# mulns/AccFlow

Measured on AMD Instinct MI355X. Metric: frame-pairs/s (estimator pair-evals/s), AccFlow(RAFT) 7-frame 480x1024 backward accumulation, higher is better.
Workload: dtype f32 (direct-kernel operands split into 2 fp16 terms - activations kept pre-split in HBM as fp16 hi+lo, 4 B per element; other kernels 3 bf16 terms; f32 accumulate)

## Files before the change

accflow_amd/_lib.py:

```python
import ctypes
import os
import threading

_HERE = os.path.dirname(os.path.abspath(__file__))
LIB_PATH = os.environ.get("ACCFLOW_HIP_LIB") or os.path.join(_HERE, "lib", "libaccflow_hip.so")

ABI_VERSION = 20
c_f = ctypes.c_void_p
c_ll = ctypes.c_longlong
c_i = ctypes.c_int


class ConvSrc(ctypes.Structure):
    _fields_ = [
        ("ptr", c_f), ("bs", c_ll),
        ("C", c_i), ("Hs", c_i), ("Ws", c_i),
        ("step", c_i), ("oy", c_i), ("ox", c_i),
        ("KH", c_i), ("KW", c_i), ("padH", c_i), ("padW", c_i),
        ("reserved", c_i),
    ]


MAX_SRC = 4

# ... 48 lines not shown
    "accflow_conv_pack_patch": [c_f, c_f, c_i, c_i, c_i, c_i, c_f, c_f],
    "accflow_conv_pack_patch16": [c_f, c_f, c_i, c_i, c_i, c_i, c_f, c_f, c_f],
    "accflow_conv_pack_split16": [c_f, c_f, c_i, c_i, c_i, c_i, c_f, c_f, c_f],
    "accflow_conv_multi_pack_elems": [c_i, c_i, ctypes.POINTER(c_i), ctypes.POINTER(c_i), ctypes.POINTER(c_i)],
    "accflow_conv_pack_multi16": [ctypes.POINTER(c_f), c_f, c_i, c_i, ctypes.POINTER(c_i), ctypes.POINTER(c_i), ctypes.POINTER(c_i),
                                  c_f, c_f, c_f],
    "accflow_conv2d_f32": [ctypes.POINTER(ConvDesc), c_f],
    "accflow_conv_stat_slots": [ctypes.POINTER(ConvDesc)],
    "accflow_conv_in_norm_supported": [ctypes.POINTER(ConvDesc)],
    "accflow_conv_plan_query": [ctypes.POINTER(ConvDesc), ctypes.POINTER(c_i), c_i],
    "accflow_conv_gru16_supported": [],
    "accflow_instance_stats_finalize_f32": [c_f, c_i, c_f, c_i, c_i, ctypes.c_float, c_f],
    "accflow_instance_norm_apply_f32": [c_f, c_f, c_i, c_f, c_f, c_f, c_i, c_i, c_i, ctypes.c_float, c_i, c_f],
    "accflow_instance_norm_apply_s16_f32": [c_f, c_f, c_i, c_f, c_f, c_f, c_f, c_ll, c_f, c_i, c_i, c_i, ctypes.c_float, c_i, c_f],
    "accflow_instance_norm_apply_s16res_f32": [c_f, c_f, c_i, c_f, c_f, c_ll, c_f, c_f, c_ll, c_f, c_i, c_i, c_i, ctypes.c_float, c_f],
    "accflow_instance_stats_finalize_sub_f32": [c_f, c_i, c_i, c_i, c_f, c_i, c_i, ctypes.c_float, c_f],
    "accflow_instance_norm_apply_s16proj_f32": [c_f, c_f, c_i, c_f, c_ll, c_f, c_i, c_i, c_i, c_f, c_f, c_ll, c_f, c_i, c_i, c_i,
                                                ctypes.c_float, c_f],
    "accflow_get_occ_s16": [c_f, c_ll, c_f, c_ll, c_f, c_ll, c_f, c_ll, c_f, c_i, c_i, c_i, c_i, c_i, c_f],
    "accflow_blend_s16": [c_f, c_f, c_f, c_f, c_ll, c_f, c_i, c_i, c_i, c_f],
    "accflow_deform_columns_s16": [c_f, c_ll, c_f, c_ll, c_f, c_ll, c_i, c_f, c_ll, c_f, c_i, c_i, c_i, c_i, c_i, c_i, c_i, c_i, c_f],
    "accflow_corr_volume_f32": [c_f, c_f, c_f, c_f, c_f, c_f, c_i, c_i, c_i, c_i, c_f],
    "accflow_corr_volume_ws_bytes": [c_i, c_i, c_i],
    "accflow_corr_volume_split_f32": [c_f, c_f, c_f, c_f, c_f, c_f, c_f, c_i, c_i, c_i, c_i, c_i, c_f],
    "accflow_corr_lookup_f32": [c_f, c_f, c_f, c_f, c_f, c_f, c_ll, c_i, c_i, c_i, c_f],
    "accflow_corr_disp_supported": [c_i, c_i],
    "accflow_corr_disp_level_elems": [c_i, c_i, c_i],
    "accflow_corr_volume_disp_f32": [c_f, c_f, c_f, c_f, c_f, c_f, c_f, c_i, c_f, c_i, c_i, c_i, c_i, c_f],
    "accflow_corr_pack_bytes": [c_i, c_i, c_i],
    "accflow_corr_pack_f32": [c_f, c_f, c_i, c_f, c_i, c_i, c_i, c_i, c_f],
    "accflow_corr_volume_disp_packed_f32": [c_f, c_i, ctypes.POINTER(c_i), ctypes.POINTER(c_i), c_f, c_f, c_f, c_f, c_i, c_f, c_i, c_i, c_i,
                                            c_i, c_f],
    "accflow_corr_disp_pool_f32": [c_f, c_f, c_f, c_f, c_i, c_i, c_i, c_f],
    "accflow_corr_lookup_disp_f32": [c_f, c_f, c_f, c_f, c_f, c_f, c_ll, c_i, c_i, c_i, c_f],
    "accflow_corr_lookup_disp_s16": [c_f, c_f, c_f, c_f, c_f, c_f, c_ll, c_f, c_i, c_i, c_i, c_f],
    "accflow_corr_alt_pyramid_elems": [c_i, c_i, c_i],
    "accflow_corr_alt_pyramid_f32": [c_f, c_f, c_i, c_i, c_i, c_i, c_f],
    "accflow_corr_lookup_alt_f32": [c_f, c_i, c_f, c_f, c_f, c_ll, c_i, c_i, c_i, c_i, c_f],
    "accflow_corr_lookup_alt_s16": [c_f, c_i, c_f, c_f, c_f, c_ll, c_f, c_i, c_i, c_i, c_i, c_f],
    "accflow_corr_lookup_convc1_kpad": [],
    "accflow_corr_lookup_convc1_s16": [c_f, c_f, c_f, c_f, c_f, c_f, c_f, c_f, c_f, c_ll, c_f, c_ll, c_i, c_f, c_i, c_i, c_i, c_i, c_f],
    "accflow_flow_from_coords_s16": [c_f, c_f, c_ll, c_f, c_ll, c_f, c_ll, c_f, c_ll, c_i, c_f, c_i, c_i, c_i, c_i, c_f],
    "accflow_convex_upsample_f32": [c_f, c_ll, c_f, c_ll, c_f, c_i, c_i, c_i, c_f],
    "accflow_backwarp_f32": [c_f, c_ll, c_f, c_ll, c_f, c_ll, c_i, c_i, c_i, c_i, c_f],
    "accflow_compose_flow_f32": [c_f, c_ll, c_f, c_ll, c_f, c_ll, c_i, c_i, c_i, c_f],
    "accflow_get_occ_f32": [c_f, c_ll, c_f, c_ll, c_f, c_ll, c_f, c_ll, c_i, c_i, c_i, c_i, c_i, c_f],
    "accflow_downflow8_f32": [c_f, c_f, c_i, c_i, c_i, c_i, c_f],
    "accflow_forward_interpolate_f32": [c_f, c_f, c_i, c_i, c_i, c_f],
    "accflow_instance_norm_f32": [c_f, c_f, c_f, c_i, c_i, c_i, ctypes.c_float, c_i, c_f],
    "accflow_split_tanh_relu_f32": [c_f, c_f, c_ll, c_f, c_ll, c_i, c_i, c_i, c_i, c_f],
    "accflow_split_tanh_relu_idx_f32": [c_f, c_i, ctypes.POINTER(c_i), c_f, c_ll, c_f, c_ll, c_i, c_i, c_i, c_i, c_f],
    "accflow_coords_grid_f32": [c_f, c_f, c_i, c_i, c_i, c_f],
    "accflow_flow_from_coords_f32": [c_f, c_f, c_ll, c_f, c_ll, c_f, c_i, c_i, c_i, c_i, c_f],
    "accflow_deform_columns_f32": [c_f, c_ll, c_f, c_ll, c_f, c_ll, c_f, c_i, c_i, c_i, c_i, c_i, c_i, c_i, c_i, c_f],
    "accflow_conv_pack_all_f32": [c_f, c_f, c_i, c_i, c_i, c_i, c_i, c_i, c_i, c_f, c_f, c_f, c_f, c_f, c_f, c_f, c_f],
    "accflow_tap_sum_f32": [c_f, c_f, c_f, c_ll, c_f, c_ll, c_i, c_i, c_i, c_i, c_i, c_i, c_i, c_i, c_i, c_i, c_f],
    "accflow_tap_sum_parts_f32": [c_f, c_i, c_ll, c_ll, c_f, c_f, c_ll, c_f, c_ll, c_i, c_i, c_i, c_i, c_i, c_i, c_i, c_i, c_i, c_i, c_f],
    "accflow_blend_f32": [c_f, c_f, c_f, c_f, c_i, c_i, c_i, c_f],
    "accflow_activation_f32": [c_f, c_ll, c_i, c_i, c_i, c_i, c_f],
    "accflow_copy_f32": [c_f, c_ll, c_f, c_ll, c_i, c_i, c_i, c_f],
    "accflow_gma_attention_f32": [c_f, c_f, c_i, c_i, c_i, ctypes.c_float, c_f],
    "accflow_gma_attention_ws_bytes": [c_i, c_i, c_i],
    "accflow_gma_attention_t_f32": [c_f, c_f, c_f, c_i, c_i, c_i, c_i, c_i, ctypes.c_float, c_f],
    "accflow_gma_aggregate_ws_bytes": [c_i, c_i, c_i],
    "accflow_gma_attention_s16_ws_bytes": [c_i, c_i, c_i],
    "accflow_gma_attention_s16": [c_f, c_f, c_f, c_f, c_i, c_i, c_i, c_i, ctypes.c_float, c_f],
# ... 59 lines not shown
```

accflow_amd/csrc/conv2d.hip:

```cpp
#include "conv_common.h"

namespace {

__global__ void conv_pack_patch_kernel(const float* __restrict__ w, const float* __restrict__ scale, int Cout, int Cin,
                                       int T, int CoutPad, unsigned short* __restrict__ wp, int f16,
                                       const float* __restrict__ wscale16, int octs = 2,
                                       const float* __restrict__ gptr = nullptr) {
  const int nstep = (Cin + 8 * octs - 1) / (8 * octs) * T;
  const long long per_term = (long long)nstep * octs * CoutPad * 8;
  const long long idx = (long long)blockIdx.x * blockDim.x + threadIdx.x;
  if (idx >= per_term) return;
  const int q = (int)(idx & 7);
  long long r = idx >> 3;
  const int ch = (int)(r % CoutPad); r /= CoutPad;
  const int o = (int)(r % octs); r /= octs;
  const int step = (int)r, cc = step / T, tap = step % T;
  const int c = cc * 8 * octs + o * 8 + q;
  float val = 0.0f;
  if (c < Cin && ch < Cout) {
    val = w[((long long)ch * Cin + c) * T + tap];
    if (scale) val *= scale[ch];
    if (gptr) val *= gptr[0];
  }
  float rr = val;
// ... 27 lines not shown
  const int k = (int)(idx / CoutPad), o = (int)(idx % CoutPad);
  const int T = KH * KW, K = Cin * T;
  float val = 0.0f;
  if (k < K && o < Cout) {
    const int c = k / T, t = k % T;
    val = kmajor ? w[(long long)k * Cout + o] : w[((long long)o * Cin + c) * T + t];
    if (scale) val *= scale[o];
    val *= cscale;
    if (gptr) val *= gptr[0];
  }
  const long long per_term = (long long)Kpad * CoutPad;
  const long long dst = ((long long)(k / 8) * CoutPad + o) * 8 + (k % 8);
  float r = val;
  if (wscale16) {
    r = val * (ldexpf(1.0f, -ACCFLOW_F16_ASHIFT) / wscale16[o]);
#pragma unroll
    for (int t = 0; t < 3; ++t) {
      const _Float16 hq = t < 2 ? (_Float16)r : (_Float16)0.0f;
      ws[t * per_term + dst] = __builtin_bit_cast(unsigned short, hq);
      r -= (float)hq;
    }
    return;
  }
#pragma unroll
  for (int t = 0; t < 3; ++t) {
    const __bf16 b = (__bf16)r;
    ws[t * per_term + dst] = __builtin_bit_cast(unsigned short, b);
    r -= (float)b;
  }
}

__global__ __launch_bounds__(256) void conv_pack_kmajor_kernel(const float* __restrict__ w, int Cout, int K, int Kpad,
                                                               int CoutPad, u32x4* __restrict__ ws, float cscale, int f16,
                                                               int* guard) {
  const long long idx = (long long)blockIdx.x * 256 + threadIdx.x;
  if (idx >= (long long)(Kpad / 8) * CoutPad) return;
  const int k8 = (int)(idx / CoutPad), o = (int)(idx % CoutPad);
  float x[8];
#pragma unroll
  for (int j = 0; j < 8; ++j) {
    const int k = k8 * 8 + j;
    x[j] = (k < K && o < Cout) ? w[(long long)k * Cout + o] * cscale : 0.0f;
  }
  const long long per_term = (long long)(Kpad / 8) * CoutPad;
  if (f16) {
    u32x4 t2[2];
    bool bad = false;
    split8_f16<0>(x, t2, bad, 1.0f);
    if (bad && guard) atomicOr(guard, 1);
    ws[idx] = t2[0];
    ws[per_term + idx] = t2[1];
  } else {
    u32x4 t3[3];
    split8_bf16<3, 0>(x, t3);
#pragma unroll
    for (int t = 0; t < 3; ++t) ws[t * per_term + idx] = t3[t];
  }
}

template <int CO>
__global__ __launch_bounds__(256) void conv2d_small_cout_kernel(const accflow_conv_desc d) {
  __shared__ float red[4][CO][64];
  const int tid = threadIdx.x, lane = tid & 63;
  const int q = __builtin_amdgcn_readfirstlane(tid >> 6);
  const int OHW = d.OH * d.OW;
  const int Ptot = d.B * OHW;
  const int p = blockIdx.x * 64 + lane;
  const bool pvalid = p < Ptot;
  const int pb = pvalid ? p / OHW : 0;
// ... 530 lines not shown
      d.in0 = reinterpret_cast<const float*>(bsplit);
      d.wpatch = wsplit;
      if (f16) { d.wpatch16 = wsplit; d.guard = guard; d.acc_scale = 1.0f / (fs * fs); }
      if (!lvl1) return 1;
      d.out2 = lvl1 + (long long)b * ((P + 127) / 128) * 128 * (H8 >> 1) * (W8 >> 1);
      const int rc = accflow_launch_corr_disp_direct(d, st);
      if (rc) return rc;
      if (lvl1_done) *lvl1_done = 1;
      continue;
    }
    if (disp) {
      const int rc = accflow_launch_corr_disp_bf16s(d, st);
      if (rc) return rc;
      continue;
    }
    const int rc = accflow_conv2d_f32(&d, st);
    if (rc) return rc;
  }
  return (int)hipGetLastError();
}

extern "C" long long accflow_corr_pack_bytes(int C, int H8, int W8) {
  return 3LL * accflow_conv_kpad(C, 1, 1) * accflow_conv_coutpad(H8 * W8) * 2;
}

extern "C" int accflow_corr_pack_f32(const float* fmaps, void* packs, int mode, int* guard, int F, int C, int H8, int W8,
                                     void* stream) {
  if (!fmaps || !packs || F <= 0 || C < 16 || (C % 16) || (W8 & 1) || !accflow_corr_disp_supported(H8, W8)) return 1;
  if (mode != ACCFLOW_CONV_BF16X3 && mode != ACCFLOW_CONV_BF16X6 && mode != ACCFLOW_CONV_F16X3) return 1;
  const int P = H8 * W8, Kpad = accflow_conv_kpad(C, 1, 1), CoutPad = accflow_conv_coutpad(P);
  const bool f16 = mode == ACCFLOW_CONV_F16X3;
  const float fs = f16 ? ldexpf(1.0f, ACCFLOW_F16_ASHIFT) : 1.0f;
  const long long n = (long long)Kpad * CoutPad, bytes = accflow_corr_pack_bytes(C, H8, W8);
  for (int f = 0; f < F; ++f)
    hipLaunchKernelGGL(conv_pack_kmajor_kernel, dim3(cdiv(n / 8, 256)), dim3(256), 0, as_stream(stream),
                       fmaps + (long long)f * C * P, P, C, Kpad, CoutPad,
                       reinterpret_cast<u32x4*>(reinterpret_cast<char*>(packs) + f * bytes), fs, f16 ? 1 : 0, guard);
  ACCFLOW_RETURN_LAUNCH_STATUS();
}

int accflow_corr_disp_pool_from(const float* lvl0, float* lvl1, float* lvl2, float* lvl3, int B, int H8, int W8, int first,
                                hipStream_t st);

extern "C" int accflow_corr_volume_disp_packed_f32(const void* packs, int F, const int* idx1, const int* idx2, float* lvl0,
                                                   float* lvl1, float* lvl2, float* lvl3, int mode, int* guard, int B,
                                                   int C, int H8, int W8, void* stream) {
  if (!packs || F <= 0 || !idx1 || !idx2 || !lvl0 || !lvl1 || !lvl2 || !lvl3 || B <= 0 || C < 16 || (C % 16) || (W8 & 1) ||
      !accflow_corr_disp_supported(H8, W8))
    return 1;
  for (int b = 0; b < B; ++b)
    if (idx1[b] < 0 || idx2[b] < 0 || idx1[b] >= F || idx2[b] >= F) return 1;
  if (mode != ACCFLOW_CONV_BF16X3 && mode != ACCFLOW_CONV_BF16X6 && mode != ACCFLOW_CONV_F16X3) return 1;
  hipStream_t st = as_stream(stream);
  const int P = H8 * W8, Kpad = accflow_conv_kpad(C, 1, 1), CoutPad = accflow_conv_coutpad(P);
  const bool f16 = mode == ACCFLOW_CONV_F16X3;
  const float fs = f16 ? ldexpf(1.0f, ACCFLOW_F16_ASHIFT) : 1.0f;
  const long long bytes = accflow_corr_pack_bytes(C, H8, W8);
  const long long pair0 = (long long)((P + 127) / 128) * 128 * P, pair1 = (long long)((P + 127) / 128) * 128 * (H8 >> 1) * (W8 >> 1);
  for (int b = 0; b < B; ++b) {
    const char* a = reinterpret_cast<const char*>(packs) + idx1[b] * bytes;
    const char* t = reinterpret_cast<const char*>(packs) + idx2[b] * bytes;
    accflow_conv_desc d = {};
    d.in0 = reinterpret_cast<const float*>(t);
    d.C0 = C; d.B = 1; d.H = H8; d.W = W8; d.OH = H8; d.OW = W8; d.KH = 1; d.KW = 1; d.stride = 1;
    d.Cout = P; d.Kpad = Kpad; d.CoutPad = CoutPad;
    d.out = lvl0 + b * pair0; d.out_bs = pair0; d.out2 = lvl1 + b * pair1;
    d.mode = mode; d.wpatch = a;
    if (f16) { d.wpatch16 = a; d.guard = guard; }
    d.acc_scale = (1.0f / sqrtf((float)C)) / (fs * fs);
    const int rc = accflow_launch_corr_disp_direct(d, st);
    if (rc) return rc;
  }
  return accflow_corr_disp_pool_from(lvl0, lvl1, lvl2, lvl3, B, H8, W8, 1, st);
}

int accflow_gma_aggregate_conv(const float* attnT, const float* v, const float* fmap, const float* gamma, float* out,
                               long long out_bs, void* ws, int mode, int* guard, int B, int D, int H, int W, hipStream_t st) {
  const int P = H * W;
  const int Kpad = accflow_conv_kpad(P, 1, 1), CoutPad = accflow_conv_coutpad(D);
  if (mode == ACCFLOW_CONV_F16X3 && B == 1 && P >= 16) {
    unsigned short* wpatch16 = reinterpret_cast<unsigned short*>(ws);
    float* wscale16 = reinterpret_cast<float*>(wpatch16 + accflow_conv_patch_elems(D, P, 1, 1));
    float* kws = wscale16 + CoutPad;
    const long long n = accflow_conv_patch_elems(D, P, 1, 1) / 3;
    hipLaunchKernelGGL(conv_row_scale16_kernel, dim3(CoutPad), dim3(256), 0, st, v, nullptr, D, P, wscale16, gamma);
    hipLaunchKernelGGL(conv_pack_patch_kernel, dim3(cdiv(n, 256)), dim3(256), 0, st, v, nullptr, D, P, 1, CoutPad, wpatch16, 1,
                       wscale16, 2, gamma);
    accflow_conv_desc d = {};
    d.in0 = attnT; d.in0_bs = (long long)P * P; d.C0 = P;
    d.B = 1; d.H = H; d.W = W; d.OH = H; d.OW = W; d.KH = 1; d.KW = 1; d.stride = 1;
    d.Cout = D; d.Kpad = Kpad; d.CoutPad = CoutPad;
    d.out = out; d.out_bs = out_bs;
    d.act = ACCFLOW_ACT_NONE; d.epi = ACCFLOW_EPI_ACCUM; d.e0 = fmap; d.e0_bs = (long long)D * P;
    d.wpatch = wpatch16; d.wpatch16 = wpatch16; d.wscale16 = wscale16; d.mode = mode; d.guard = guard;
    d.kws = kws; d.kws_elems = 8LL * D * P;
    conv_plan p;
    if (conv_plan_direct(d, D > 64 ? 2 : 1, false, p)) return 1;
    return accflow_launch_conv_direct(d, p, st);
  }
  if (D <= 32) return 1;
  unsigned short* wsplit = reinterpret_cast<unsigned short*>(ws);
  int* ktab = reinterpret_cast<int*>(wsplit + 3LL * Kpad * CoutPad * B);
  float* wscale16 = reinterpret_cast<float*>(reinterpret_cast<char*>(ktab) + (long long)Kpad * 16);
  float* kws = wscale16 + (((long long)B * CoutPad + 3) & ~3LL);
  hipLaunchKernelGGL(conv_ktab_kernel, dim3(cdiv(Kpad, 256)), dim3(256), 0, st, P, Kpad, reinterpret_cast<int4*>(ktab));
// ... 216 lines not shown
```

accflow_amd/csrc/conv2d_direct.hip:

```cpp
#include "conv2d_direct_kernel.h"

namespace {

__global__ __launch_bounds__(256) void conv_ksplit_reduce_kernel(const accflow_conv_desc d, int Z) {
  const int OHW = d.OH * d.OW;
  const long long n = (long long)d.B * d.Cout * OHW;
  const long long i = (long long)blockIdx.x * 256 + threadIdx.x;
  if (i >= n) return;
  const int px = (int)(i % OHW);
  const int ch = (int)((i / OHW) % d.Cout);
  const int b = (int)(i / ((long long)OHW * d.Cout));
  float v = d.kws[i];
  for (int z = 1; z < Z; ++z) v += d.kws[(long long)z * n + i];
  v = fmaf(v, d.wscale16 ? d.wscale16[(d.wsplit_bs ? (long long)b * d.CoutPad : 0) + ch] : 1.0f, d.bias ? d.bias[ch] : 0.0f);
  if (d.pre && (d.epi == ACCFLOW_EPI_GRU_ZR || d.epi == ACCFLOW_EPI_GRU_Q)) v += d.pre[b * d.pre_bs + (long long)ch * OHW + px];
  v = apply_act(v, d.act);
  const long long o = (long long)ch * OHW + px;
  const int half = d.Cout >> 1;
  if (d.cb) {
    const int blk = ch / d.cb;
    const long long oc = (long long)(ch - blk * d.cb) * OHW + px;
    const float r = d.epi == ACCFLOW_EPI_ACCUM ? d.e0[b * d.e0_bs + blk * d.e0_cbs + oc] + v : v;
    d.out[b * d.out_bs + blk * d.out_cbs + oc] = r;
    return;
// ... 453 lines not shown
    if (mr > -INFINITY) s += part[((long long)r * P + i) * 2 + 1] * expf(mr - m);
  }
  stats[2 * i] = m;
  stats[2 * i + 1] = 1.0f / s;
}

int accflow_launch_gma_attn(const void* kpack, const void* qpack, float* part, float* stats, void* out16, float acc_scale, int P,
                            int D, int Ppad, hipStream_t st) {
  gma_attn_args a;
  a.kpack = kpack; a.qpack = qpack; a.part = part; a.stats = stats; a.out16 = reinterpret_cast<unsigned*>(out16);
  a.acc_scale = acc_scale; a.P = P; a.D = D; a.Ppad = Ppad;
  const int nb = cdiv(P, 128);
  hipLaunchKernelGGL((gma_attn_gemm_kernel<0>), dim3(nb * nb), dim3(256), 0, st, a);
  hipLaunchKernelGGL(gma_attn_stats_kernel, dim3(cdiv(P, 256)), dim3(256), 0, st, part, stats, P, nb);
  hipLaunchKernelGGL((gma_attn_gemm_kernel<1>), dim3(nb * nb), dim3(256), 0, st, a);
  ACCFLOW_RETURN_LAUNCH_STATUS();
}

int accflow_launch_gma_attn_stats(const void* kpack, const void* qpack, float* part, float* stats, float acc_scale, int P, int D,
                                  int Ppad, hipStream_t st) {
  gma_attn_args a;
  a.kpack = kpack; a.qpack = qpack; a.part = part; a.stats = stats; a.out16 = nullptr;
  a.acc_scale = acc_scale; a.P = P; a.D = D; a.Ppad = Ppad;
  const int nb = cdiv(P, 128);
  hipLaunchKernelGGL((gma_attn_gemm_kernel<0>), dim3(nb * nb), dim3(256), 0, st, a);
  hipLaunchKernelGGL(gma_attn_stats_kernel, dim3(cdiv(P, 256)), dim3(256), 0, st, part, stats, P, nb);
  ACCFLOW_RETURN_LAUNCH_STATUS();
}

constexpr int CRING_SLOT_CHUNKS = 2 * 2 * 2 * 128;
#ifndef ACCFLOW_CORR_ABL
#define ACCFLOW_CORR_ABL 0
#endif
__global__ __launch_bounds__(256, 2) void corr_disp_ring_kernel(const accflow_conv_desc d) {
  constexpr int TC = 2, TP = 2;
  constexpr int CRING_SLOTS = 3;
  constexpr int RING_BYTES = CRING_SLOTS * CRING_SLOT_CHUNKS * 16;
  constexpr int ST_BYTES = DISP2_LDS_BYTES;
  __shared__ __attribute__((aligned(16))) unsigned char smem[RING_BYTES > ST_BYTES ? RING_BYTES : ST_BYTES];
  u32x4* ring = reinterpret_cast<u32x4*>(smem);
#ifdef ACCFLOW_KPROF
  const unsigned long long tL0 = __builtin_amdgcn_s_memrealtime();
#endif
  const int tid = threadIdx.x, lane = tid & 63;
  const int wave = __builtin_amdgcn_readfirstlane(tid >> 6);
  const int wc = wave >> 1, wp = wave & 1;
  const int l31 = lane & 31, kh = lane >> 5;
  const int P = d.OH * d.OW;
  const int npb = (P + 127) >> 7, percol = (npb + 7) >> 3;
  const int xcd = blockIdx.x & 7, seq = blockIdx.x >> 3;
  const int pb = xcd + 8 * (seq % percol), qt = seq / percol;
  if (pb >= npb) return;
  const int ncx = (d.OW + 63) >> 6;
  const int yo = qt / ncx, xc = qt - yo * ncx;
  const int cblk0 = pb * 128;
  const int nstep = d.Kpad / 16;
  const unsigned oct_bytes = (unsigned)d.CoutPad * 16u, term_bytes = (unsigned)(d.Kpad / 8) * oct_bytes;
  const __amdgpu_buffer_rsrc_t ra = __builtin_amdgcn_make_buffer_rsrc(const_cast<void*>(d.wpatch16), 0, (int)(2 * term_bytes), 0x00020000);
  const __amdgpu_buffer_rsrc_t rb = __builtin_amdgcn_make_buffer_rsrc(const_cast<float*>(d.in0), 0, (int)(2 * term_bytes), 0x00020000);
  unsigned pvoff[4];
  int prow[4];
#pragma unroll
  for (int i = 0; i < 4; ++i) {
    const int id = wave * 4 + i;
    const int isb = id >> 3, row = (id >> 1) & 3, half = id & 1;
    prow[i] = row;
    if (!isb) {
      pvoff[i] = (unsigned)(cblk0 + half * 64 + lane) * 16u;
    } else {
// ... 53 lines not shown
          if (ACCFLOW_CORR_ABL & 2) acc[tc][tp][pr] += __builtin_bit_cast(float, __builtin_bit_cast(u32x4, A[PA[pr]][tc])[0] ^ __builtin_bit_cast(u32x4, Bf[PB[pr]][tp])[1]);
          else acc[tc][tp] = dir_mfma<true>(A[PA[pr]][tc], Bf[PB[pr]][tp], acc[tc][tp]);
        }
  }
  __syncthreads();
  if ((ACCFLOW_CORR_ABL & 8) && acc[0][0][0] != 12345.678f) return;
#ifdef ACCFLOW_KPROF
  __builtin_amdgcn_sched_barrier(0);
  const unsigned long long tL1 = __builtin_amdgcn_s_memrealtime();
#endif
  corr_disp_store2(d, acc, reinterpret_cast<float*>(smem), reinterpret_cast<int*>(smem) + 64 * DISP_PITCH,
                   reinterpret_cast<float*>(smem + DISP_LDS_BYTES), d.out2, cblk0, yo, xc, wc, wp, lane, wave, tid);
#ifdef ACCFLOW_KPROF
  __builtin_amdgcn_sched_barrier(0);
  const unsigned long long tL2 = __builtin_amdgcn_s_memrealtime();
  asm volatile("s_waitcnt vmcnt(0)" ::: "memory");
  if (tid == 0) {
    const int slot = (blockIdx.x & 4095) * 16;
    g_kprof[slot + 8] = tL1 - tL0;
    g_kprof[slot + 9] = tL2 - tL1;
    g_kprof[slot + 11] = __builtin_amdgcn_s_memrealtime() - tL0;
    g_kprof[slot + 10] = 1;
  }
#endif
}

int accflow_launch_corr_disp_direct(const accflow_conv_desc& d, hipStream_t st) {
  const int P = d.OH * d.OW, npb = cdiv(P, 128);
  if (!d.out2) return 1;
  const int nqt = cdiv(d.OH, 2) * cdiv(d.OW, 64);
  dim3 grid(8 * ((npb + 7) / 8) * nqt);
  static const bool ringk = [] { const char* e = getenv("ACCFLOW_CORR_GEMM"); return !(e && e[0] == 'r'); }();
  if (d.mode == ACCFLOW_CONV_F16X3 && d.wpatch16 && ringk) {
    hipLaunchKernelGGL(corr_disp_ring_kernel, grid, dim3(256), 0, st, d);
  } else if (d.mode == ACCFLOW_CONV_F16X3 && d.wpatch16) hipLaunchKernelGGL((corr_disp_gemm_kernel<2, true>), grid, dim3(256), 0, st, d);
  else if (d.mode == ACCFLOW_CONV_BF16X3) hipLaunchKernelGGL((corr_disp_gemm_kernel<2, false>), grid, dim3(256), 0, st, d);
  else hipLaunchKernelGGL((corr_disp_gemm_kernel<3, false>), grid, dim3(256), 0, st, d);
  ACCFLOW_RETURN_LAUNCH_STATUS();
}

int accflow_launch_conv_direct(const accflow_conv_desc& d, const conv_plan& p, hipStream_t st) {
  if (!p.ch0) return launch_conv_direct(d, p, st);
  accflow_conv_desc part[2];
  conv_tail_split(d, p.ch0, part[0], part[1]);
  for (int i = 0; i < 2; ++i) {
    conv_plan pp;
    int rc = conv_plan_part(part[i], p, i == 1, pp);
    if (!rc) rc = launch_conv_direct(part[i], pp, st);
    if (rc) return rc;
  }
  return 0;
}

#ifdef ACCFLOW_KPROF
#define ACCFLOW_DIRECT_UNITY
#include "conv2d_direct_v_s16.hip"
#include "conv2d_direct_v_s16tg.hip"
#include "conv2d_direct_v_s16k.hip"
#include "conv2d_direct_v_s16k9.hip"
#include "conv2d_direct_v_f16.hip"
#include "conv2d_direct_v_f16n.hip"
#include "conv2d_direct_v_bf16x6.hip"
#include "conv2d_direct_v_bf16x3.hip"
#include "conv2d_direct_v_bf16n.hip"
extern "C" int accflow_debug_occupancy(int* out) {
  int n = 0;
  hipOccupancyMaxActiveBlocksPerMultiprocessor(&out[n++], conv2d_direct_bf16s_kernel<2, 3>, 256, 0);
  hipOccupancyMaxActiveBlocksPerMultiprocessor(&out[n++], conv2d_direct_bf16s_kernel<2, 2, true>, 256, 0);
  hipOccupancyMaxActiveBlocksPerMultiprocessor(&out[n++], conv2d_direct_bf16s_kernel<1, 3>, 256, 0);
  hipDeviceProp_t pr; hipGetDeviceProperties(&pr, 0);
// ... 13 lines not shown
```

accflow_amd/csrc/corr_disp.hip:

```cpp
#include "common.h"

namespace {

constexpr int R = 4, WIN = 2 * R + 2;
constexpr unsigned OOB = 0x40000000u;

__global__ __launch_bounds__(256) void corr_disp_pool_kernel(const float* __restrict__ in, float* __restrict__ out,
                                                             int Hi, int Wi, int W8, int P, int lsrc) {
  const int p = blockIdx.x * 256 + threadIdx.x;
  if (p >= P) return;
  const int Ho = Hi >> 1, Wo = Wi >> 1;
  const int dy = blockIdx.y / Wo, dx = blockIdx.y - dy * Wo;
  const int y1 = p / W8, x1 = p - y1 * W8;
  int yo = dy + (y1 >> (lsrc + 1)), xo = dx + (x1 >> (lsrc + 1));
  if (yo >= Ho) yo -= Ho;
  if (xo >= Wo) xo -= Wo;
  int sy0 = 2 * yo - (y1 >> lsrc), sx0 = 2 * xo - (x1 >> lsrc);
  int sy1 = sy0 + 1, sx1 = sx0 + 1;
  if (sy0 < 0) sy0 += Hi;
  if (sy1 < 0) sy1 += Hi;
  if (sx0 < 0) sx0 += Wi;
  if (sx1 < 0) sx1 += Wi;
  const int PB = (P + 127) >> 7;
  const float* src = in + (((long long)blockIdx.z * PB + (p >> 7)) * Hi * Wi) * 128 + (p & 127);
  const float a = src[(long long)(sy0 * Wi + sx0) * 128], b = src[(long long)(sy0 * Wi + sx1) * 128];
  const float c = src[(long long)(sy1 * Wi + sx0) * 128], d = src[(long long)(sy1 * Wi + sx1) * 128];
  out[((((long long)blockIdx.z * PB + (p >> 7)) * Ho * Wo) + blockIdx.y) * 128 + (p & 127)] = (((a + b) + c) + d) * 0.25f;
}

typedef unsigned lu32x4 __attribute__((ext_vector_type(4)));
template <int PF, bool OUT16 = false>
__global__ __launch_bounds__(64) void corr_lookup_disp_kernel(const float* __restrict__ l0, const float* __restrict__ l1,
                                                               const float* __restrict__ l2, const float* __restrict__ l3,
                                                               const float* __restrict__ coords, float* __restrict__ out,
                                                               long long out_bs, int H8, int W8, int* guard = nullptr) {
  const int P = H8 * W8;
  const int lane = threadIdx.x & 63;
  const int lvl = blockIdx.z;
  const int b = blockIdx.y;
  const int pix = blockIdx.x * 64 + lane;
  const bool active = pix < P;
  const int pc = active ? pix : 0;

  const float* vol = lvl == 0 ? l0 : lvl == 1 ? l1 : lvl == 2 ? l2 : l3;
  const int Hl = H8 >> lvl, Wl = W8 >> lvl;
  const int PB = (P + 127) >> 7, pblk = (blockIdx.x * 64) >> 7;
  const long long slab = (long long)Hl * Wl * 128;
  const __amdgpu_buffer_rsrc_t rsrc = __builtin_amdgcn_make_buffer_rsrc(
      const_cast<float*>(vol + ((long long)b * PB + pblk) * slab), 0, (int)(slab * 4), 0x00020000);

  const float inv = 1.0f / (float)(1 << lvl);
  float cx = coords[((long long)b * 2 + 0) * P + pc] * inv;
  float cy = coords[((long long)b * 2 + 1) * P + pc] * inv;
  cx = fminf(fmaxf(cx, -1.0e6f), 1.0e6f);
  cy = fminf(fmaxf(cy, -1.0e6f), 1.0e6f);
  const float fx0 = floorf(cx), fy0 = floorf(cy);
  const float ax = cx - fx0, ay = cy - fy0;
  const int xs = (int)fx0 - R, ys = (int)fy0 - R;
  const float w00 = (1.0f - ax) * (1.0f - ay), w01 = ax * (1.0f - ay), w10 = (1.0f - ax) * ay, w11 = ax * ay;

  const int y1 = pc / W8, x1 = pc - y1 * W8;
  const int y1l = y1 >> lvl, x1l = x1 >> lvl;
// ... 55 lines not shown
  for (int j = 0; j < 2 * R + 1; ++j) {
    if (j + PF < WIN) load_row(j + PF, rows[(j + PF) % (PF + 1)]);
    const float (&r0)[WIN] = rows[j % (PF + 1)];
    const float (&r1)[WIN] = rows[(j + 1) % (PF + 1)];
    if constexpr (OUT16) {
#pragma unroll
      for (int i = 0; i < 2 * R + 1; ++i) {
        const int n = j * 9 + i;
        buf[n & 7] = blend4(r0[i], r0[i + 1], r1[i], r1[i + 1]);
        if ((n & 7) == 7 || n == 80) flush(n >> 3, (n & 7) + 1);
      }
    } else if (active) {
#pragma unroll
      for (int i = 0; i < 2 * R + 1; ++i) {
        o[(long long)(i * 9 + j) * P] = blend4(r0[i], r0[i + 1], r1[i], r1[i + 1]);
      }
    }
  }
  if constexpr (OUT16) {
    if (bad && guard) atomicOr(guard, 1);
  }
}

}

extern "C" int accflow_corr_disp_supported(int H8, int W8) {
  return H8 >= 8 && W8 >= 8 && H8 < 65536 && W8 < 65536 && (long long)H8 * W8 * 512 <= (long long)OOB;
}

extern "C" long long accflow_corr_disp_level_elems(int H8, int W8, int level) {
  return (long long)(((long long)H8 * W8 + 127) / 128) * 128 * (H8 >> level) * (W8 >> level);
}

int accflow_corr_disp_pool_from(const float* lvl0, float* lvl1, float* lvl2, float* lvl3, int B, int H8, int W8, int first,
                                hipStream_t st) {
  const int P = H8 * W8;
  const float* lv[4] = {lvl0, lvl1, lvl2, lvl3};
  float* dst[4] = {nullptr, lvl1, lvl2, lvl3};
  for (int l = first; l < 3; ++l) {
    const int Hi = H8 >> l, Wi = W8 >> l;
    hipLaunchKernelGGL(corr_disp_pool_kernel, dim3(cdiv(P, 256), (Hi >> 1) * (Wi >> 1), B), dim3(256), 0, st, lv[l],
                       dst[l + 1], Hi, Wi, W8, P, l);
  }
  ACCFLOW_RETURN_LAUNCH_STATUS();
}

extern "C" int accflow_corr_disp_pool_f32(const float* lvl0, float* lvl1, float* lvl2, float* lvl3, int B, int H8,
                                          int W8, void* stream) {
  if (!lvl0 || !lvl1 || !lvl2 || !lvl3 || B <= 0 || !accflow_corr_disp_supported(H8, W8)) return 1;
  return accflow_corr_disp_pool_from(lvl0, lvl1, lvl2, lvl3, B, H8, W8, 0, as_stream(stream));
}

extern "C" int accflow_corr_lookup_disp_f32(const float* lvl0, const float* lvl1, const float* lvl2,
                                            const float* lvl3, const float* coords, float* out, long long out_bs,
                                            int B, int H8, int W8, void* stream) {
  if (!lvl0 || !lvl1 || !lvl2 || !lvl3 || !coords || !out || B <= 0 || !accflow_corr_disp_supported(H8, W8)) return 1;
  hipLaunchKernelGGL(corr_lookup_disp_kernel<1>, dim3(cdiv((long long)H8 * W8, 64), B, 4), dim3(64), 0, as_stream(stream),
                     lvl0, lvl1, lvl2, lvl3, coords, out, out_bs, H8, W8);
  ACCFLOW_RETURN_LAUNCH_STATUS();
}

extern "C" int accflow_corr_lookup_disp_s16(const float* lvl0, const float* lvl1, const float* lvl2, const float* lvl3,
                                            const float* coords, void* out16, long long out16_bs, int* guard, int B, int H8,
                                            int W8, void* stream) {
  if (!lvl0 || !lvl1 || !lvl2 || !lvl3 || !coords || !out16 || B <= 0 || !accflow_corr_disp_supported(H8, W8)) return 1;
  hipLaunchKernelGGL((corr_lookup_disp_kernel<1, true>), dim3(cdiv((long long)H8 * W8, 64), B, 4), dim3(64), 0,
                     as_stream(stream), lvl0, lvl1, lvl2, lvl3, coords, reinterpret_cast<float*>(out16), out16_bs, H8, W8, guard);
  ACCFLOW_RETURN_LAUNCH_STATUS();
}
```

include/accflow_hip.h:

```cpp
#ifndef ACCFLOW_HIP_H
#define ACCFLOW_HIP_H

#ifdef __cplusplus
extern "C" {
#endif

#define ACCFLOW_ABI_VERSION 20

enum { ACCFLOW_ACT_NONE = 0, ACCFLOW_ACT_RELU = 1, ACCFLOW_ACT_SIGMOID = 2, ACCFLOW_ACT_TANH = 3 };

enum {
  ACCFLOW_EPI_STORE = 0,
  ACCFLOW_EPI_RES_RELU = 1,
  ACCFLOW_EPI_GRU_ZR = 2,
  ACCFLOW_EPI_GRU_Q = 3,
  ACCFLOW_EPI_ACCUM = 4,
  ACCFLOW_EPI_TAPGEMM = 5
};

enum {
  ACCFLOW_CONV_F32 = 0,
  ACCFLOW_CONV_BF16X3 = 2,
  ACCFLOW_CONV_BF16X6 = 3,
  ACCFLOW_CONV_F16X3 = 4
// ... 86 lines not shown
                              const int* KW, void* wpatch16, float* wscale16, void* stream);

int accflow_conv2d_f32(const accflow_conv_desc* desc, void* stream);
int accflow_conv_stat_slots(const accflow_conv_desc* desc);
int accflow_conv_in_norm_supported(const accflow_conv_desc* desc);
int accflow_conv_plan_query(const accflow_conv_desc* desc, int* out, int n);
int accflow_conv_gru16_supported(void);

int accflow_corr_volume_f32(const float* fmap1, const float* fmap2, float* lvl0, float* lvl1,
                            float* lvl2, float* lvl3, int B, int C, int H8, int W8, void* stream);

long long accflow_corr_volume_ws_bytes(int C, int H8, int W8);
int accflow_corr_volume_split_f32(const float* fmap1, const float* fmap2, float* lvl0, float* lvl1,
                                  float* lvl2, float* lvl3, void* ws, int mode, int B, int C, int H8,
                                  int W8, void* stream);

int accflow_corr_lookup_f32(const float* lvl0, const float* lvl1, const float* lvl2,
                            const float* lvl3, const float* coords, float* out, long long out_bs,
                            int B, int H8, int W8, void* stream);

int accflow_corr_disp_supported(int H8, int W8);
long long accflow_corr_disp_level_elems(int H8, int W8, int level);
int accflow_corr_volume_disp_f32(const float* fmap1, const float* fmap2, float* lvl0, float* lvl1,
                                 float* lvl2, float* lvl3, void* ws, int mode, int* guard, int B, int C,
                                 int H8, int W8, void* stream);
long long accflow_corr_pack_bytes(int C, int H8, int W8);
int accflow_corr_pack_f32(const float* fmaps, void* packs, int mode, int* guard, int F, int C, int H8, int W8,
                          void* stream);
int accflow_corr_volume_disp_packed_f32(const void* packs, int F, const int* idx1, const int* idx2, float* lvl0,
                                        float* lvl1, float* lvl2, float* lvl3, int mode, int* guard, int B, int C, int H8,
                                        int W8, void* stream);
int accflow_corr_disp_pool_f32(const float* lvl0, float* lvl1, float* lvl2, float* lvl3, int B, int H8,
                               int W8, void* stream);
int accflow_corr_lookup_disp_f32(const float* lvl0, const float* lvl1, const float* lvl2,
                                 const float* lvl3, const float* coords, float* out, long long out_bs,
                                 int B, int H8, int W8, void* stream);

int accflow_corr_lookup_disp_s16(const float* lvl0, const float* lvl1, const float* lvl2, const float* lvl3,
                                 const float* coords, void* out16, long long out16_bs, int* guard, int B, int H8,
                                 int W8, void* stream);

long long accflow_corr_alt_pyramid_elems(int C, int H8, int W8);
int accflow_corr_alt_pyramid_f32(const float* fmaps, float* pyr, int F, int C, int H8, int W8, void* stream);
int accflow_corr_lookup_alt_f32(const float* pyr, int F, const int* idx, const float* coords, float* out, long long out_bs,
                                int B, int C, int H8, int W8, void* stream);
int accflow_corr_lookup_alt_s16(const float* pyr, int F, const int* idx, const float* coords, void* out16, long long out16_bs,
                                int* guard, int B, int C, int H8, int W8, void* stream);

int accflow_corr_lookup_convc1_kpad(void);
int accflow_corr_lookup_convc1_s16(const float* lvl0, const float* lvl1, const float* lvl2, const float* lvl3,
                                   const float* coords, const void* wpatch16, const float* wscale16, const float* bias,
                                   void* out16, long long out16_bs, float* out, long long out_bs, int act, int* guard,
                                   int B, int H8, int W8, int Cout, void* stream);

int accflow_convex_upsample_f32(const float* flow, long long flow_bs, const float* mask,
                                long long mask_bs, float* out, int B, int H8, int W8, void* stream);

int accflow_backwarp_f32(const float* img, long long img_bs, const float* flow, long long flow_bs,
                         float* out, long long out_bs, int B, int C, int H, int W, void* stream);

int accflow_compose_flow_f32(const float* step, long long step_bs, const float* acc, long long acc_bs,
                             float* out, long long out_bs, int B, int H, int W, void* stream);

int accflow_get_occ_f32(const float* flow, long long flow_bs, const float* i1, long long i1_bs,
                        const float* i2, long long i2_bs, float* out, long long out_bs, int B, int C,
                        int H, int W, int binary, void* stream);
// ... 123 lines not shown
```

Measured before the change: 533.4.

## Batch correlation pair launches and fuse pyramid pooling levels two and three

Correlation-volume computation for all frame pairs now runs in one launch per 16 pairs. The pair indices are passed through kernel arguments and read from the kernarg segment, replacing one launch per pair. The per-frame pack kernel is batched over grid.y, and a new fused kernel builds pool levels 2 and 3 in one pass, which removes an intermediate launch and a re-read of level 2. The goals are less launch overhead, better GPU fill from concurrent pairs, and less memory traffic, at the cost of a larger kernarg struct and more complex index math in the pooling kernel.

```diff
diff --git a/accflow_amd/_lib.py b/accflow_amd/_lib.py
--- a/accflow_amd/_lib.py
+++ b/accflow_amd/_lib.py
@@ -104,6 +104,7 @@
     "accflow_corr_volume_disp_packed_f32": [c_f, c_i, ctypes.POINTER(c_i), ctypes.POINTER(c_i), c_f, c_f, c_f, c_f, c_i, c_f, c_i, c_i, c_i,
                                             c_i, c_f],
     "accflow_corr_disp_pool_f32": [c_f, c_f, c_f, c_f, c_i, c_i, c_i, c_f],
+    "accflow_corr_disp_pool_levels_f32": [c_f, c_f, c_f, c_f, c_i, c_i, c_i, c_i, c_i, c_f],
     "accflow_corr_lookup_disp_f32": [c_f, c_f, c_f, c_f, c_f, c_f, c_ll, c_i, c_i, c_i, c_f],
     "accflow_corr_lookup_disp_s16": [c_f, c_f, c_f, c_f, c_f, c_f, c_ll, c_f, c_i, c_i, c_i, c_f],
     "accflow_corr_alt_pyramid_elems": [c_i, c_i, c_i],
diff --git a/accflow_amd/csrc/conv2d.hip b/accflow_amd/csrc/conv2d.hip
--- a/accflow_amd/csrc/conv2d.hip
+++ b/accflow_amd/csrc/conv2d.hip
@@ -83,9 +83,11 @@
 
 __global__ __launch_bounds__(256) void conv_pack_kmajor_kernel(const float* __restrict__ w, int Cout, int K, int Kpad,
                                                                int CoutPad, u32x4* __restrict__ ws, float cscale, int f16,
-                                                               int* guard) {
+                                                               int* guard, long long w_ms = 0, long long ws_ms = 0) {
   const long long idx = (long long)blockIdx.x * 256 + threadIdx.x;
   if (idx >= (long long)(Kpad / 8) * CoutPad) return;
+  w += blockIdx.y * w_ms;
+  ws += blockIdx.y * ws_ms;
   const int k8 = (int)(idx / CoutPad), o = (int)(idx % CoutPad);
   float x[8];
 #pragma unroll
@@ -682,15 +684,20 @@
   const bool f16 = mode == ACCFLOW_CONV_F16X3;
   const float fs = f16 ? ldexpf(1.0f, ACCFLOW_F16_ASHIFT) : 1.0f;
   const long long n = (long long)Kpad * CoutPad, bytes = accflow_corr_pack_bytes(C, H8, W8);
-  for (int f = 0; f < F; ++f)
-    hipLaunchKernelGGL(conv_pack_kmajor_kernel, dim3(cdiv(n / 8, 256)), dim3(256), 0, as_stream(stream),
-                       fmaps + (long long)f * C * P, P, C, Kpad, CoutPad,
-                       reinterpret_cast<u32x4*>(reinterpret_cast<char*>(packs) + f * bytes), fs, f16 ? 1 : 0, guard);
+  for (int f0 = 0; f0 < F; f0 += 65535) {
+    const int nf = F - f0 < 65535 ? F - f0 : 65535;
+    hipLaunchKernelGGL(conv_pack_kmajor_kernel, dim3(cdiv(n / 8, 256), nf), dim3(256), 0, as_stream(stream),
+                       fmaps + (long long)f0 * C * P, P, C, Kpad, CoutPad,
+                       reinterpret_cast<u32x4*>(reinterpret_cast<char*>(packs) + f0 * bytes), fs, f16 ? 1 : 0, guard,
+                       (long long)C * P, bytes / 16);
+  }
   ACCFLOW_RETURN_LAUNCH_STATUS();
 }
 
 int accflow_corr_disp_pool_from(const float* lvl0, float* lvl1, float* lvl2, float* lvl3, int B, int H8, int W8, int first,
                                 hipStream_t st);
+int accflow_launch_corr_disp_pairs(const accflow_conv_desc& d, long long pack_bytes, const int* idx1, const int* idx2, int npair,
+                                   hipStream_t st);
 
 extern "C" int accflow_corr_volume_disp_packed_f32(const void* packs, int F, const int* idx1, const int* idx2, float* lvl0,
                                                    float* lvl1, float* lvl2, float* lvl3, int mode, int* guard, int B,
@@ -707,20 +714,16 @@
   const float fs = f16 ? ldexpf(1.0f, ACCFLOW_F16_ASHIFT) : 1.0f;
   const long long bytes = accflow_corr_pack_bytes(C, H8, W8);
   const long long pair0 = (long long)((P + 127) / 128) * 128 * P, pair1 = (long long)((P + 127) / 128) * 128 * (H8 >> 1) * (W8 >> 1);
-  for (int b = 0; b < B; ++b) {
-    const char* a = reinterpret_cast<const char*>(packs) + idx1[b] * bytes;
-    const char* t = reinterpret_cast<const char*>(packs) + idx2[b] * bytes;
-    accflow_conv_desc d = {};
-    d.in0 = reinterpret_cast<const float*>(t);
-    d.C0 = C; d.B = 1; d.H = H8; d.W = W8; d.OH = H8; d.OW = W8; d.KH = 1; d.KW = 1; d.stride = 1;
-    d.Cout = P; d.Kpad = Kpad; d.CoutPad = CoutPad;
-    d.out = lvl0 + b * pair0; d.out_bs = pair0; d.out2 = lvl1 + b * pair1;
-    d.mode = mode; d.wpatch = a;
-    if (f16) { d.wpatch16 = a; d.guard = guard; }
-    d.acc_scale = (1.0f / sqrtf((float)C)) / (fs * fs);
-    const int rc = accflow_launch_corr_disp_direct(d, st);
-    if (rc) return rc;
-  }
+  accflow_conv_desc d = {};
+  d.in0 = reinterpret_cast<const float*>(packs);
+  d.C0 = C; d.B = 1; d.H = H8; d.W = W8; d.OH = H8; d.OW = W8; d.KH = 1; d.KW = 1; d.stride = 1;
+  d.Cout = P; d.Kpad = Kpad; d.CoutPad = CoutPad;
+  d.out = lvl0; d.out_bs = pair0; d.out2 = lvl1; d.out2_bs = pair1;
+  d.mode = mode; d.wpatch = packs;
+  if (f16) { d.wpatch16 = packs; d.guard = guard; }
+  d.acc_scale = (1.0f / sqrtf((float)C)) / (fs * fs);
+  const int rc = accflow_launch_corr_disp_pairs(d, bytes, idx1, idx2, B, st);
+  if (rc) return rc;
   return accflow_corr_disp_pool_from(lvl0, lvl1, lvl2, lvl3, B, H8, W8, 1, st);
 }
 
diff --git a/accflow_amd/csrc/conv2d_direct.hip b/accflow_amd/csrc/conv2d_direct.hip
--- a/accflow_amd/csrc/conv2d_direct.hip
+++ b/accflow_amd/csrc/conv2d_direct.hip
@@ -509,9 +509,27 @@
 #ifndef ACCFLOW_CORR_ABL
 #define ACCFLOW_CORR_ABL 0
 #endif
-__global__ __launch_bounds__(256, 2) void corr_disp_ring_kernel(const accflow_conv_desc d) {
+constexpr int CORR_BATCH_MAX = 16;
+struct corr_batch_args {
+  accflow_conv_desc d;
+  long long pack_bytes;
+  int ia[CORR_BATCH_MAX], it[CORR_BATCH_MAX];
+};
+__global__ __launch_bounds__(256, 2) void corr_disp_ring_kernel(const corr_batch_args a) {
   constexpr int TC = 2, TP = 2;
   constexpr int CRING_SLOTS = 3;
+  accflow_conv_desc d = a.d;
+  {
+    typedef const __attribute__((address_space(4))) int* kint_ptr;
+    const kint_ptr k = (kint_ptr)((const __attribute__((address_space(4))) char*)__builtin_amdgcn_kernarg_segment_ptr() +
+                                  __builtin_offsetof(corr_batch_args, ia));
+    const int pair = blockIdx.y;
+    const int fa = k[pair], ft = k[CORR_BATCH_MAX + pair];
+    d.wpatch16 = reinterpret_cast<const char*>(a.d.wpatch16) + fa * a.pack_bytes;
+    d.in0 = reinterpret_cast<const float*>(reinterpret_cast<const char*>(a.d.wpatch16) + ft * a.pack_bytes);
+    d.out = a.d.out + pair * a.d.out_bs;
+    d.out2 = a.d.out2 + pair * a.d.out2_bs;
+  }
   constexpr int RING_BYTES = CRING_SLOTS * CRING_SLOT_CHUNKS * 16;
   constexpr int ST_BYTES = DISP2_LDS_BYTES;
   __shared__ __attribute__((aligned(16))) unsigned char smem[RING_BYTES > ST_BYTES ? RING_BYTES : ST_BYTES];
@@ -631,10 +649,45 @@
   dim3 grid(8 * ((npb + 7) / 8) * nqt);
   static const bool ringk = [] { const char* e = getenv("ACCFLOW_CORR_GEMM"); return !(e && e[0] == 'r'); }();
   if (d.mode == ACCFLOW_CONV_F16X3 && d.wpatch16 && ringk) {
-    hipLaunchKernelGGL(corr_disp_ring_kernel, grid, dim3(256), 0, st, d);
+    corr_batch_args a = {};
+    a.d = d;
+    a.pack_bytes = reinterpret_cast<const char*>(d.in0) - reinterpret_cast<const char*>(d.wpatch16);
+    a.ia[0] = 0; a.it[0] = 1;
+    hipLaunchKernelGGL(corr_disp_ring_kernel, grid, dim3(256), 0, st, a);
   } else if (d.mode == ACCFLOW_CONV_F16X3 && d.wpatch16) hipLaunchKernelGGL((corr_disp_gemm_kernel<2, true>), grid, dim3(256), 0, st, d);
   else if (d.mode == ACCFLOW_CONV_BF16X3) hipLaunchKernelGGL((corr_disp_gemm_kernel<2, false>), grid, dim3(256), 0, st, d);
   else hipLaunchKernelGGL((corr_disp_gemm_kernel<3, false>), grid, dim3(256), 0, st, d);
+  ACCFLOW_RETURN_LAUNCH_STATUS();
+}
+
+int accflow_launch_corr_disp_pairs(const accflow_conv_desc& d, long long pack_bytes, const int* idx1, const int* idx2,
+                                   int npair, hipStream_t st) {
+  const int P = d.OH * d.OW, npb = cdiv(P, 128);
+  if (!d.out2 || npair <= 0) return 1;
+  const int nqt = cdiv(d.OH, 2) * cdiv(d.OW, 64);
+  static const bool ringk = [] { const char* e = getenv("ACCFLOW_CORR_GEMM"); return !(e && e[0] == 'r'); }();
+  const char* packs = reinterpret_cast<const char*>(d.mode == ACCFLOW_CONV_F16X3 ? d.wpatch16 : d.wpatch);
+  if (!(d.mode == ACCFLOW_CONV_F16X3 && d.wpatch16 && ringk)) {
+    for (int b = 0; b < npair; ++b) {
+      accflow_conv_desc e = d;
+      e.in0 = reinterpret_cast<const float*>(packs + idx2[b] * pack_bytes);
+      e.wpatch = packs + idx1[b] * pack_bytes;
+      if (d.wpatch16) e.wpatch16 = e.wpatch;
+      e.out = d.out + b * d.out_bs; e.out2 = d.out2 + b * d.out2_bs;
+      const int rc = accflow_launch_corr_disp_direct(e, st);
+      if (rc) return rc;
+    }
+    return 0;
+  }
+  for (int b0 = 0; b0 < npair; b0 += CORR_BATCH_MAX) {
+    const int nb = npair - b0 < CORR_BATCH_MAX ? npair - b0 : CORR_BATCH_MAX;
+    corr_batch_args a = {};
+    a.d = d;
+    a.d.out = d.out + b0 * d.out_bs; a.d.out2 = d.out2 + b0 * d.out2_bs;
+    a.pack_bytes = pack_bytes;
+    for (int b = 0; b < nb; ++b) { a.ia[b] = idx1[b0 + b]; a.it[b] = idx2[b0 + b]; }
+    hipLaunchKernelGGL(corr_disp_ring_kernel, dim3(8 * ((npb + 7) / 8) * nqt, nb), dim3(256), 0, st, a);
+  }
   ACCFLOW_RETURN_LAUNCH_STATUS();
 }
 
diff --git a/accflow_amd/csrc/corr_disp.hip b/accflow_amd/csrc/corr_disp.hip
--- a/accflow_amd/csrc/corr_disp.hip
+++ b/accflow_amd/csrc/corr_disp.hip
@@ -28,6 +28,49 @@
   out[((((long long)blockIdx.z * PB + (p >> 7)) * Ho * Wo) + blockIdx.y) * 128 + (p & 127)] = (((a + b) + c) + d) * 0.25f;
 }
 
+__global__ __launch_bounds__(256) void corr_disp_pool23_kernel(const float* __restrict__ l1, float* __restrict__ l2,
+                                                               float* __restrict__ l3, int H8, int W8, int P) {
+  const int p = blockIdx.x * 256 + threadIdx.x;
+  if (p >= P) return;
+  const int H1 = H8 >> 1, W1 = W8 >> 1, H2 = H8 >> 2, W2 = W8 >> 2, H3 = H8 >> 3, W3 = W8 >> 3;
+  const int W3c = (W2 + 1) >> 1;
+  const int cy = blockIdx.y / W3c, cx = blockIdx.y - cy * W3c;
+  const int y1 = p / W8, x1 = p - y1 * W8;
+  int Y3 = cy, X3 = cx;
+  if (cy < H3) { Y3 = cy + (y1 >> 3); if (Y3 >= H3) Y3 -= H3; }
+  if (cx < W3) { X3 = cx + (x1 >> 3); if (X3 >= W3) X3 -= W3; }
+  const int PB = (P + 127) >> 7;
+  const long long blk = (long long)blockIdx.z * PB + (p >> 7);
+  const float* src = l1 + blk * H1 * W1 * 128 + (p & 127);
+  float* dst2 = l2 + blk * H2 * W2 * 128 + (p & 127);
+  float v[2][2];
+#pragma unroll
+  for (int i = 0; i < 2; ++i)
+#pragma unroll
+    for (int j = 0; j < 2; ++j) {
+      const int yo = 2 * Y3 + i, xo = 2 * X3 + j;
+      v[i][j] = 0.0f;
+      if (yo < H2 && xo < W2) {
+        int sy0 = 2 * yo - (y1 >> 1), sx0 = 2 * xo - (x1 >> 1);
+        int sy1 = sy0 + 1, sx1 = sx0 + 1;
+        if (sy0 < 0) sy0 += H1;
+        if (sy1 < 0) sy1 += H1;
+        if (sx0 < 0) sx0 += W1;
+        if (sx1 < 0) sx1 += W1;
+        const float a = src[(long long)(sy0 * W1 + sx0) * 128], b = src[(long long)(sy0 * W1 + sx1) * 128];
+        const float c = src[(long long)(sy1 * W1 + sx0) * 128], d = src[(long long)(sy1 * W1 + sx1) * 128];
+        v[i][j] = __fmul_rn(__fadd_rn(__fadd_rn(__fadd_rn(a, b), c), d), 0.25f);
+        int dy = yo - (y1 >> 2), dx = xo - (x1 >> 2);
+        if (dy < 0) dy += H2;
+        if (dx < 0) dx += W2;
+        dst2[(long long)(dy * W2 + dx) * 128] = v[i][j];
+      }
+    }
+  if (cy < H3 && cx < W3)
+    l3[(blk * H3 * W3 + cy * W3 + cx) * 128 + (p & 127)] =
+        __fmul_rn(__fadd_rn(__fadd_rn(__fadd_rn(v[0][0], v[0][1]), v[1][0]), v[1][1]), 0.25f);
+}
+
 typedef unsigned lu32x4 __attribute__((ext_vector_type(4)));
 template <int PF, bool OUT16 = false>
 __global__ __launch_bounds__(64) void corr_lookup_disp_kernel(const float* __restrict__ l0, const float* __restrict__ l1,
@@ -149,23 +192,37 @@
   return (long long)(((long long)H8 * W8 + 127) / 128) * 128 * (H8 >> level) * (W8 >> level);
 }
 
-int accflow_corr_disp_pool_from(const float* lvl0, float* lvl1, float* lvl2, float* lvl3, int B, int H8, int W8, int first,
-                                hipStream_t st) {
+static int corr_disp_pool_levels(const float* lvl0, float* lvl1, float* lvl2, float* lvl3, int B, int H8, int W8, int first,
+                                 int fused, hipStream_t st) {
   const int P = H8 * W8;
   const float* lv[4] = {lvl0, lvl1, lvl2, lvl3};
   float* dst[4] = {nullptr, lvl1, lvl2, lvl3};
-  for (int l = first; l < 3; ++l) {
+  for (int l = first; l < (fused ? 1 : 3); ++l) {
     const int Hi = H8 >> l, Wi = W8 >> l;
     hipLaunchKernelGGL(corr_disp_pool_kernel, dim3(cdiv(P, 256), (Hi >> 1) * (Wi >> 1), B), dim3(256), 0, st, lv[l],
                        dst[l + 1], Hi, Wi, W8, P, l);
   }
+  if (fused)
+    hipLaunchKernelGGL(corr_disp_pool23_kernel, dim3(cdiv(P, 256), (((H8 >> 2) + 1) >> 1) * (((W8 >> 2) + 1) >> 1), B),
+                       dim3(256), 0, st, lvl1, lvl2, lvl3, H8, W8, P);
   ACCFLOW_RETURN_LAUNCH_STATUS();
+}
+
+int accflow_corr_disp_pool_from(const float* lvl0, float* lvl1, float* lvl2, float* lvl3, int B, int H8, int W8, int first,
+                                hipStream_t st) {
+  return corr_disp_pool_levels(lvl0, lvl1, lvl2, lvl3, B, H8, W8, first, 1, st);
 }
 
 extern "C" int accflow_corr_disp_pool_f32(const float* lvl0, float* lvl1, float* lvl2, float* lvl3, int B, int H8,
                                           int W8, void* stream) {
   if (!lvl0 || !lvl1 || !lvl2 || !lvl3 || B <= 0 || !accflow_corr_disp_supported(H8, W8)) return 1;
   return accflow_corr_disp_pool_from(lvl0, lvl1, lvl2, lvl3, B, H8, W8, 0, as_stream(stream));
+}
+
+extern "C" int accflow_corr_disp_pool_levels_f32(const float* lvl0, float* lvl1, float* lvl2, float* lvl3, int B, int H8,
+                                                 int W8, int first, int fused, void* stream) {
+  if (!lvl0 || !lvl1 || !lvl2 || !lvl3 || B <= 0 || first < 0 || first > 1 || !accflow_corr_disp_supported(H8, W8)) return 1;
+  return corr_disp_pool_levels(lvl0, lvl1, lvl2, lvl3, B, H8, W8, first, fused, as_stream(stream));
 }
 
 extern "C" int accflow_corr_lookup_disp_f32(const float* lvl0, const float* lvl1, const float* lvl2,
diff --git a/include/accflow_hip.h b/include/accflow_hip.h
--- a/include/accflow_hip.h
+++ b/include/accflow_hip.h
@@ -142,6 +142,8 @@
                                         int W8, void* stream);
 int accflow_corr_disp_pool_f32(const float* lvl0, float* lvl1, float* lvl2, float* lvl3, int B, int H8,
                                int W8, void* stream);
+int accflow_corr_disp_pool_levels_f32(const float* lvl0, float* lvl1, float* lvl2, float* lvl3, int B, int H8, int W8,
+                                      int first, int fused, void* stream);
 int accflow_corr_lookup_disp_f32(const float* lvl0, const float* lvl1, const float* lvl2,
                                  const float* lvl3, const float* coords, float* out, long long out_bs,
                                  int B, int H8, int W8, void* stream);
```

New measurement: 531.7. Within noise of the previous version (-0.3%).
